# neuronest/custom-alphazero

Measured on AMD Instinct MI355X. Metric: self-play games/s (Connect-4 6x7, 100 sims/move), higher is better.
Workload: dtype fp32-accurate network (fp16 MFMA, two-term split operands, 3 products) / f64 PUCT

## Files before the change

### custom-alphazero_amd/csrc/az_tower16.hip

```cpp
#include <algorithm>
#include <cmath>
#include <cstring>
#include <functional>
#include <type_traits>

#include "az_nn.h"
#include "az_tree.h"
#include "az_kloop_asm.h"
#include "az_chess.h"

namespace az {

typedef _Float16 t_h8 __attribute__((ext_vector_type(8)));
typedef float t_f4 __attribute__((ext_vector_type(4)));

namespace {

constexpr float kRange = 32752.f;
constexpr int kPitch = 544;
constexpr int kZeroRows = 8;
__device__ __forceinline__ bool pix_ok(int yx) { return ((yx >> 8) & 255) != 127; }
__device__ __forceinline__ int pix_row(int yx, int HW, int W) {
  return pix_ok(yx) ? (yx >> 16) * HW + ((yx >> 8) & 255) * W + (yx & 255) : (yx & 7);
}

#ifdef AZ_T16_STAMPS
constexpr int kStampBlocks = 4096, kStamps = 64;
__device__ unsigned long long g_t16_stamps[kStampBlocks][kStamps];
#define T16_STAMP(k)                                                             \
  if (threadIdx.x == 0 && blockIdx.x < kStampBlocks) {                           \
    g_t16_stamps[blockIdx.x][k] = __builtin_amdgcn_s_memtime();                  \
  }
#define T16_RSTAMP(k)                                                            \
  if (threadIdx.x == 0 && blockIdx.x < kStampBlocks) {                           \
    g_t16_stamps[blockIdx.x][k] = __builtin_amdgcn_s_memrealtime();              \
  }
__device__ unsigned long long g_t16_wstamps[kStampBlocks][8][5];
#define T16_WSTAMP(d, k)                                                          \
  if ((d) == 1 && (threadIdx.x & 63) == 0 && blockIdx.x < kStampBlocks) {        \
    g_t16_wstamps[blockIdx.x][threadIdx.x >> 6][k] = __builtin_amdgcn_s_memtime(); \
    if ((k) == 0)                                                                 \
      g_t16_wstamps[blockIdx.x][threadIdx.x >> 6][4] =                            \
          (unsigned)__builtin_amdgcn_s_getreg((31 << 11) | 4);                    \
  }
#define T16_STAMP4(k)                      \
  if (threadIdx.x == 256 && blockIdx.x < kStampBlocks) {                         \
    g_t16_stamps[blockIdx.x][k] = __builtin_amdgcn_s_memtime();                  \
  }
#else
#define T16_STAMP4(k)
#define T16_WSTAMP(d, k)
#define T16_STAMP(k)
#define T16_RSTAMP(k)
#endif

template <typename T>
__device__ __forceinline__ const __attribute__((address_space(1))) T* gbl(const T* p) {
  return (const __attribute__((address_space(1))) T*)p;
}
template <typename T>
__device__ __forceinline__ T gld(const T* p) {
  static_assert(sizeof(T) % 4 == 0, "32-bit words");
  typedef unsigned int V __attribute__((ext_vector_type(sizeof(T) / 4)));
  return __builtin_bit_cast(T, *(const __attribute__((address_space(1))) V*)p);
}


__device__ __forceinline__ void split_u4(const float4 v, uint2& t0, uint2& t1) {
  const float x[4] = {v.x, v.y, v.z, v.w};
  uint32_t p[2], q[2];
#pragma unroll
  for (int i = 0; i < 2; ++i) {
    p[i] = pk_f16(x[2 * i], x[2 * i + 1]);
    const az_h2 h = __builtin_bit_cast(az_h2, p[i]);
    q[i] = pk_f16(x[2 * i] - (float)h[0], x[2 * i + 1] - (float)h[1]);
  }
  t0 = make_uint2(p[0], p[1]);
  t1 = make_uint2(q[0], q[1]);
}
__device__ __forceinline__ void split_u8(const float (&x)[8], uint4& t0, uint4& t1) {
  uint2 a0, a1, b0, b1;
  split_u4(make_float4(x[0], x[1], x[2], x[3]), a0, a1);
  split_u4(make_float4(x[4], x[5], x[6], x[7]), b0, b1);
  t0 = make_uint4(a0.x, a0.y, b0.x, b0.y);
  t1 = make_uint4(a1.x, a1.y, b1.x, b1.y);
}

template <int CTRL>
__device__ __forceinline__ float dpp_f(float v) {
  return __builtin_bit_cast(float, __builtin_amdgcn_update_dpp(0, __builtin_bit_cast(int, v), CTRL, 0xf, 0xf, false));
}
template <typename F>
__device__ __forceinline__ float wreduce(float v, F op) {
  v = op(v, dpp_f<0xB1>(v));
  v = op(v, dpp_f<0x4E>(v));
  v = op(v, dpp_f<0x124>(v));
  v = op(v, dpp_f<0x128>(v));
  const float r0 = __builtin_bit_cast(float, __builtin_amdgcn_readlane(__builtin_bit_cast(int, v), 0));
  const float r1 = __builtin_bit_cast(float, __builtin_amdgcn_readlane(__builtin_bit_cast(int, v), 16));
  const float r2 = __builtin_bit_cast(float, __builtin_amdgcn_readlane(__builtin_bit_cast(int, v), 32));
  const float r3 = __builtin_bit_cast(float, __builtin_amdgcn_readlane(__builtin_bit_cast(int, v), 48));
  return op(op(r0, r1), op(r2, r3));
}
__device__ __forceinline__ float wsum(float v) {
  return wreduce(v, [](float a, float b) { return a + b; });
}
__device__ __forceinline__ float wmax(float v) {
  return wreduce(v, [](float a, float b) { return fmaxf(a, b); });
}

__device__ __forceinline__ int range_exp(float m) {
  int s = 0;
  while (ldexpf(m, -s) > kRange) ++s;
  return s;
}

struct TowerSmem {
  int flag[2];
  int sc[2][kTowerMaxBoards];
  unsigned bmax[kTowerMaxBoards];
};

__device__ __forceinline__ void put4(uint4* act, int r, int cq, const float4 y) {
  uint2 t0, t1;
  split_u4(y, t0, t1);
  char* q = reinterpret_cast<char*>(act) + r * kPitch + cq * 8;
  *reinterpret_cast<uint2*>(q) = t0;
  *reinterpret_cast<uint2*>(q + 256) = t1;
}

__device__ __forceinline__ float max4(const float4 v) { return fmaxf(fmaxf(v.x, v.y), fmaxf(v.z, v.w)); }
__device__ __forceinline__ float4 scale4(const float4 v, float s) {
  return make_float4(v.x * s, v.y * s, v.z * s, v.w * s);
}

template <int MBW>
__device__ __forceinline__ bool store_layer(uint4* act, int HW, int W, const int (&yx_)[MBW], int cq0, const float4 (&y)[2 * MBW],
                                            TowerSmem& sm, int par, int* sc_out, int nbrd,
                                            unsigned long long* err) {
  int row[MBW], brd[MBW];
#pragma unroll
  for (int mb = 0; mb < MBW; ++mb) {
    row[mb] = pix_ok(yx_[mb]) ? pix_row(yx_[mb], HW, W) : -1;
    brd[mb] = yx_[mb] >> 16;
    asm volatile("" : "+v"(row[mb]), "+v"(brd[mb]));
  }
  float vmax = 0.f;
#pragma unroll
  for (int i = 0; i < 2 * MBW; ++i)
    if (row[i / 2] >= 0) {
      vmax = fmaxf(vmax, max4(y[i]));
      put4(act, row[i / 2], cq0 + 4 * (i & 1), y[i]);
    }
  if (!(vmax <= kRange)) sm.flag[par] = 1;
  if (threadIdx.x == 0) sm.flag[par ^ 1] = 0;
  __syncthreads();
  if (!sm.flag[par]) return false;
  if ((int)threadIdx.x < nbrd) sm.bmax[threadIdx.x] = 0u;
  __syncthreads();
#pragma unroll
  for (int i = 0; i < 2 * MBW; ++i)
    if (row[i / 2] >= 0) atomicMax(&sm.bmax[brd[i / 2]], __float_as_uint(max4(y[i])));
  __syncthreads();
#pragma unroll
  for (int i = 0; i < 2 * MBW; ++i) {
    if (row[i / 2] < 0) continue;
    const float m = __uint_as_float(sm.bmax[brd[i / 2]]);
    if (!(m <= 3.0e38f)) continue;
    const int s = range_exp(m);
    if (s) put4(act, row[i / 2], cq0 + 4 * (i & 1), scale4(y[i], ldexpf(1.f, -s)));
  }
  if ((int)threadIdx.x < nbrd) {
    const float m = __uint_as_float(sm.bmax[threadIdx.x]);
    if (!(m <= 3.0e38f)) {
      if (err) atomicOr(err, kErrActRange);
      sc_out[threadIdx.x] = 0;
    } else {
      sc_out[threadIdx.x] = range_exp(m);
    }
  }
  __syncthreads();
  return true;
}

template <int V>
using IC = std::integral_constant<int, V>;

struct NoMid {
  __device__ void operator()() const {}
};
template <int MBW, int R, int C0 = 0, typename Mid = NoMid>
__device__ __forceinline__ void k_loop(const uint4* __restrict__ act, const uint4* __restrict__ wmain,
                                       const uint4* __restrict__ wres, t_f4 (&acc)[MBW][2],
                                       t_f4 (&accr)[MBW][2], const int (&yx_)[MBW], int H, int W,
                                       int zrow, int nq, int lane, int skw, int res_shift = 0,
                                       Mid mid = Mid{}) {
  static_assert(R == 0 || R == 4, "ring slots = k-step mod NB, NB divides 4");
  static_assert(C0 == 0 || (R == 0 && C0 == 2), "skipped chunks: the stem only, an even count");
  constexpr int PF = 1, NB = 2;
  const int gq = lane >> 4;
  int r[MBW], yx[MBW];
#pragma unroll
  for (int mb = 0; mb < MBW; ++mb) {
    yx[mb] = yx_[mb];
    asm volatile("" : "+v"(yx[mb]));
    r[mb] = pix_row(yx[mb], H * W, W);
  }
  uint4 bq[NB][4];
  const auto rs_m = __builtin_amdgcn_make_buffer_rsrc((void*)wmain, (short)0, 0x7fffffff, 0x00020000);
  const auto rs_r = __builtin_amdgcn_make_buffer_rsrc((void*)(R ? wres : wmain), (short)0, 0x7fffffff, 0x00020000);
  const int voff = ((nq * 2) * 2 * 64 + lane) * 16;
  auto load_bk = [&](int s, uint4(&dst)[4]) {
#pragma unroll
    for (int q = 0; q < 4; ++q) {
      const auto v = s < R ? __builtin_amdgcn_raw_buffer_load_b128(rs_r, voff + q * 1024, (36 + s) * 16384, 0)
                           : __builtin_amdgcn_raw_buffer_load_b128(rs_m, voff + q * 1024, (s - R) * 16384, 0);
      dst[q] = __builtin_bit_cast(uint4, v);
    }
  };

  int aaddr[MBW];
  const char* actb = reinterpret_cast<const char*>(act);
  auto set_own = [&](int lo, int hi) {
#pragma unroll
    for (int mb = 0; mb < MBW; ++mb)
      if (mb >= lo && mb < hi) aaddr[mb] = (pix_ok(yx[mb]) ? r[mb] + res_shift : zrow + (r[mb] & 7)) * kPitch + gq * 16;
  };
  auto set_tap = [&](int t, int lo, int hi) {
    const int dy = t / 3 - 1, dx = t - (t / 3) * 3 - 1;
#pragma unroll
    for (int mb = 0; mb < MBW; ++mb) {
      if (mb < lo || mb >= hi) continue;
      const int py = (yx[mb] >> 8) & 255, px = yx[mb] & 255;
      const bool ok = py + dy >= 0 && py + dy < H && px + dx >= 0 && px + dx < W;
      const int sr = r[mb] + dy * W + dx;
      aaddr[mb] = (ok ? sr : zrow + (sr & 7)) * kPitch + gq * 16;
    }
  };
  constexpr int RING = MBW > 4 ? 4 : MBW;
  constexpr bool LAG = RING == MBW && MBW > 1;
  uint4 aq[RING][2];
  auto load_a1 = [&](int chunk, int mb) {
    const char* q = actb + aaddr[mb] + 64 * chunk;
    aq[mb % RING][0] = *reinterpret_cast<const uint4*>(q);
    aq[mb % RING][1] = *reinterpret_cast<const uint4*>(q + 256);
  };
  auto kstep = [&](t_f4(&C)[MBW][2], const uint4(&b)[4], int chunk, int next_chunk, auto skc, auto skn,
                   bool first = false) {
    constexpr int SKC = decltype(skc)::value, SKN = decltype(skn)::value;
    const t_h8 B0[2] = {__builtin_bit_cast(t_h8, b[0]), __builtin_bit_cast(t_h8, b[2])};
    const t_h8 B1[2] = {__builtin_bit_cast(t_h8, b[1]), __builtin_bit_cast(t_h8, b[3])};
#pragma unroll
    for (int mb = 0; mb < MBW; ++mb) {
      const t_h8 a0 = __builtin_bit_cast(t_h8, aq[mb % RING][0]), a1 = __builtin_bit_cast(t_h8, aq[mb % RING][1]);
      if (((SKC >> mb) & 1) == 0) {
#pragma unroll
      for (int nb = 0; nb < 2; ++nb) {
        C[mb][nb] = __builtin_amdgcn_mfma_f32_16x16x32_f16(B0[nb], a1, C[mb][nb], 0, 0, 0);
        C[mb][nb] = __builtin_amdgcn_mfma_f32_16x16x32_f16(B1[nb], a0, C[mb][nb], 0, 0, 0);
        C[mb][nb] = __builtin_amdgcn_mfma_f32_16x16x32_f16(B0[nb], a0, C[mb][nb], 0, 0, 0);
      }
      }
// ... 155 lines not shown
}

#ifdef AZ_KLOOP_CC
#define AZ_KLOOP k_loop
#else
#define AZ_KLOOP k_loop_asm
#endif

template <int NT>
__device__ __forceinline__ void dma_to_lds(uint4* dst, const float* src, int n_u4, int wave, int lane) {
  if (n_u4 <= 0) return;
  const auto rsrc = __builtin_amdgcn_make_buffer_rsrc((void*)src, (short)0, n_u4 * 16, 0x00020000);
  for (int base = wave * 64; base < n_u4; base += NT) {
    const int i = base + lane;
    const unsigned voff = i < n_u4 ? (unsigned)(i * 16) : 0x80000000u;
    __builtin_amdgcn_raw_ptr_buffer_load_lds(rsrc, (__attribute__((address_space(3))) void*)(dst + base), 16,
                                             voff, 0, 0, 0);
  }
}

template <int MBT, int NWM, bool ROWS, bool DB>
__device__ __forceinline__ void tower16_tile(const TowerNet* __restrict__ net, const Board* __restrict__ boards,
                                             const float4* __restrict__ x, const uint4* __restrict__ rows,
                                             int n, int H, int W, int A, int bpw, float* __restrict__ probs,
                                             float* __restrict__ values, float4* __restrict__ feat,
                                             int first_chunk, unsigned long long* __restrict__ err,
                                             TowerLeaves lv) {
  constexpr int MBW = MBT / NWM;
  constexpr int TR = 16 * MBT;
  constexpr int NT = NWM * 256;
  extern __shared__ __attribute__((aligned(16))) uint4 act[];
  const TowerNet& T = *net;
  constexpr bool dbuf = DB;
  uint4* const bufX = act;
  uint4* const bufH = dbuf ? act + (TR + kZeroRows) * (kPitch / 16) : act;
  const int zX = TR, zH = dbuf ? -kZeroRows : TR;
  TowerSmem& sm = *reinterpret_cast<TowerSmem*>(reinterpret_cast<char*>(act) +
                                                ((dbuf ? 2 : 1) * TR + kZeroRows) * kPitch);
  float* blob = reinterpret_cast<float*>(&sm + 1);

  const int HW = H * W;
  const int b0 = blockIdx.x * bpw;
  if (b0 >= n) return;
  const int nbrd = min(bpw, n - b0);
  const int live = nbrd * HW;
  const int tid = threadIdx.x, lane = tid & 63, wave = tid >> 6;
  const int zrow = TR;
  T16_RSTAMP(22);
  T16_STAMP(0);
  const bool alt = 16 * MBT != T.tile_rows && 16 * MBT == T.alt_rows;
  const bool wpd_lds = alt ? T.alt_wpd_lds : T.wpd_lds;
  const bool wv1_lds = alt ? T.alt_wv1_lds : T.wv1_lds;
  const bool wv1_late = alt && wv1_lds;
  dma_to_lds<NT>(reinterpret_cast<uint4*>(blob), T.blob,
                 (wv1_late ? T.off_wv1 : alt ? T.alt_staged_floats : T.staged_floats) / 4, wave, lane);
  for (int i = tid; i < kZeroRows * kPitch / 16; i += NT) act[zrow * kPitch / 16 + i] = make_uint4(0u, 0u, 0u, 0u);
  if (tid < 2) sm.flag[tid] = 0;

  const int mh = wave % NWM, nq = wave / NWM, r16 = lane & 15, gq = lane >> 4;
  const int r0 = mh * MBW * 16 + r16;
  int yx[MBW];
  const bool planned = 16 * MBT == T.tile_rows || alt;
  const bool wv1_xt = T.wv1_xtile && 16 * MBT == T.tile_rows;
  const int* plan = !planned ? nullptr : alt ? T.alt_slot_pix : T.slot_pix;
  T16_STAMP(56);
#pragma unroll
  for (int mb = 0; mb < MBW; ++mb) {
    const int rr = r0 + 16 * mb;
    if (plan) {
      const int v = *gbl(plan + rr);
      yx[mb] = pix_ok(v) && (v >> 16) >= nbrd ? (127 << 8) | (pix_row(v, HW, W) & 7) : v;
    } else {
      const bool valid = rr < live;
      const int b = valid ? rr / HW : 0;
      const int p = rr - b * HW;
      yx[mb] = valid ? (b << 16) | ((p / W) << 8) | (p - (p / W) * W) : (127 << 8) | (rr & 7);
    }
  }
  const int skw = (ROWS && 16 * MBT != 128) ? 0 : !planned ? 0 : alt ? T.alt_skip[mh] : T.skip[mh];
  const int cq0 = 8 * nq + gq;
  t_f4 acc[MBW][2], accr_[MBW][2];
  auto& accr = DB ? acc : accr_;
  float4 yv[2 * MBW];

  if constexpr (ROWS) {
    char* dst = reinterpret_cast<char*>(bufH);
    auto t1_unscale = [](uint32_t w) {
      const az_h2 h = __builtin_bit_cast(az_h2, w);
      return pk_f16((float)h[0] * 0x1p-12f, (float)h[1] * 0x1p-12f);
    };
    if (lv.leaf) {
      const azc::Pos st = azc::start_pos();
      for (int i = tid; i < live * 16; i += NT) {
        const int rr = i >> 4, c4 = 16 + (i & 15), b = rr / HW, pix = rr - b * HW;
        const int s = *gbl(lv.eval_slot + b0 + b);
        const azc::Pos cur = azc::load_pos(static_cast<const az_chess_pos*>(lv.leaf)[s]);
        const bool initial = *gbl(lv.path_len + s) == 0 && *gbl(lv.initial + s) != 0;
        float f[6], v[4];
        azc::state_feats(cur, f);
        azc::full_state4(st, cur, initial, f, pix, 4 * c4, v);
        uint2 t0, t1;
        split16x4(make_float4(v[0], v[1], v[2], v[3]), t0, t1);
        char* q = dst + rr * kPitch;
        *reinterpret_cast<uint2*>(q + 8 * c4) = t0;
        *reinterpret_cast<uint2*>(q + 256 + 8 * c4) = make_uint2(t1_unscale(t1.x), t1_unscale(t1.y));
      }
    } else {
      const uint4* src = rows + (size_t)b0 * HW * 32;
#pragma unroll 4
      for (int i = tid; i < live * 32; i += NT) {
        uint4 v = gld(src + i);
        if ((i & 31) >= 16) v = make_uint4(t1_unscale(v.x), t1_unscale(v.y), t1_unscale(v.z), t1_unscale(v.w));
        *reinterpret_cast<uint4*>(dst + (i >> 5) * kPitch + (i & 31) * 16) = v;
      }
    }
#pragma unroll
    for (int mb = 0; mb < MBW; ++mb)
#pragma unroll
      for (int nb = 0; nb < 2; ++nb) acc[mb][nb] = t_f4{0.f, 0.f, 0.f, 0.f};
    __builtin_amdgcn_s_waitcnt(0);
    __syncthreads();
    if (first_chunk == 2) AZ_KLOOP<MBW, 0, 2>(bufH, T.stem_k, nullptr, acc, acc, yx, H, W, zH, nq, lane, skw);
    else AZ_KLOOP<MBW, 0, 0>(bufH, T.stem_k, nullptr, acc, acc, yx, H, W, zH, nq, lane, skw);
    if (!dbuf) __syncthreads();
  } else {
  {
    const uint4* ws = T.stem16 + (size_t)(nq * 2) * 2 * 64 + lane;
    uint4 bs2[2][4];
#pragma unroll
    for (int ks = 0; ks < 2; ++ks)
#pragma unroll
      for (int q = 0; q < 4; ++q) bs2[ks][q] = gld(ws + (size_t)ks * 1024 + q * 64);
#pragma unroll
    for (int mb = 0; mb < MBW; ++mb)
#pragma unroll
      for (int nb = 0; nb < 2; ++nb) acc[mb][nb] = t_f4{0.f, 0.f, 0.f, 0.f};
    constexpr int SG = MBW <= 4 ? MBW : MBW % 4 == 0 ? 4 : MBW % 3 == 0 ? 3 : 1;
    static_assert(MBW % SG == 0, "stem groups");
#pragma unroll
    for (int g0 = 0; g0 < MBW; g0 += SG) {
      Board bd[SG];
      if (boards) {
#pragma unroll
        for (int i = 0; i < SG; ++i) bd[i] = gld(boards + b0 + (yx[g0 + i] >> 16));
      }
#pragma unroll
      for (int ks = 0; ks < 2; ++ks) {
        const uint4(&bs)[4] = bs2[ks];
        const t_h8 B0[2] = {__builtin_bit_cast(t_h8, bs[0]), __builtin_bit_cast(t_h8, bs[2])};
        const t_h8 B1[2] = {__builtin_bit_cast(t_h8, bs[1]), __builtin_bit_cast(t_h8, bs[3])};
#pragma unroll
        for (int i = 0; i < SG; ++i) {
          const int mb = g0 + i;
          float v[8];
#pragma unroll
          for (int h = 0; h < 2; ++h) {
            const int t = 8 * ks + 2 * gq + h;
            const int dy = t / 3 - 1, dx = t - (t / 3) * 3 - 1;
            const int py = (yx[mb] >> 8) & 255, px = yx[mb] & 255;
            const bool ok = t < 9 && py + dy >= 0 && py + dy < H && px + dx >= 0 && px + dx < W;
            float4 pl = make_float4(0.f, 0.f, 0.f, 0.f);
            if (ok) {
              const int q = (py + dy) * W + px + dx;
              if (boards) {
                const uint64_t ow = q < 64 ? bd[i].own[0] : bd[i].own[1],
                               op = q < 64 ? bd[i].opp[0] : bd[i].opp[1];
                const bool o = (ow >> (q & 63)) & 1ull, e = (op >> (q & 63)) & 1ull;
                pl = make_float4(o || e ? 0.f : 1.f, o ? 1.f : 0.f, e ? 1.f : 0.f, 1.f);
              } else {
                pl = gld(x + (size_t)(b0 + (yx[mb] >> 16)) * HW + q);
              }
            }
            v[4 * h + 0] = pl.x;
            v[4 * h + 1] = pl.y;
            v[4 * h + 2] = pl.z;
            v[4 * h + 3] = pl.w;
          }
          uint4 a0, a1;
          split_u8(v, a0, a1);
#pragma unroll
          for (int nb = 0; nb < 2; ++nb) {
            acc[mb][nb] = __builtin_amdgcn_mfma_f32_16x16x32_f16(B0[nb], __builtin_bit_cast(t_h8, a1), acc[mb][nb], 0, 0, 0);
            acc[mb][nb] = __builtin_amdgcn_mfma_f32_16x16x32_f16(B1[nb], __builtin_bit_cast(t_h8, a0), acc[mb][nb], 0, 0, 0);
            acc[mb][nb] = __builtin_amdgcn_mfma_f32_16x16x32_f16(B0[nb], __builtin_bit_cast(t_h8, a0), acc[mb][nb], 0, 0, 0);
          }
        }
      }
    }
  }
  T16_STAMP(57);
  __builtin_amdgcn_s_waitcnt(0);
  T16_STAMP(58);
  __syncthreads();
  }
  T16_STAMP(1);
  {
    const float osc = ROWS ? T.stem_ks : T.stem_s;
    const float* bb = blob + T.off_stemb;
#pragma unroll
    for (int nb = 0; nb < 2; ++nb) {
      const float4 bc = *reinterpret_cast<const float4*>(bb + 32 * nq + 16 * nb + 4 * gq);
#pragma unroll
      for (int mb = 0; mb < MBW; ++mb) {
        const t_f4 a = acc[mb][nb];
        yv[mb * 2 + nb] = make_float4(fmaxf(fmaf(a[0], osc, bc.x), 0.f), fmaxf(fmaf(a[1], osc, bc.y), 0.f),
                                      fmaxf(fmaf(a[2], osc, bc.z), 0.f), fmaxf(fmaf(a[3], osc, bc.w), 0.f));
      }
    }
  }
  int par = 0;
  bool anyX = store_layer<MBW>(bufX, HW, W, yx, cq0, yv, sm, par, sm.sc[0], nbrd, err);
  bool anyH = false;
  float* red = nullptr;
  const int J = T.hidden;
  par ^= 1;
  T16_STAMP(21);

  const int depth = T.depth;
  for (int d = 0; d < depth; ++d) {
#pragma unroll
    for (int mb = 0; mb < MBW; ++mb)
#pragma unroll
      for (int nb = 0; nb < 2; ++nb) {
        acc[mb][nb] = t_f4{0.f, 0.f, 0.f, 0.f};
        accr_[mb][nb] = t_f4{0.f, 0.f, 0.f, 0.f};
      }
    T16_WSTAMP(d, 0);
    if constexpr (DB) AZ_KLOOP<MBW, 0, 0>(bufX, T.k1[d], nullptr, acc, acc, yx, H, W, zX, nq, lane, skw);
    else AZ_KLOOP<MBW, 4, 0>(bufX, T.k1[d], T.k2[d], acc, accr_, yx, H, W, zX, nq, lane, skw);
    T16_WSTAMP(d, 1);
    if (d < 4) T16_STAMP(2 + 4 * d);
    if (d < 4) T16_STAMP4(24 + 4 * d);
    if (!dbuf) __syncthreads();
    if (d < 4) T16_STAMP(40 + d);
    {
      const float osc = T.s1[d];
      const float* bb = blob + T.off_b1 + d * 128;
#pragma unroll
      for (int nb = 0; nb < 2; ++nb) {
        const float4 bc = *reinterpret_cast<const float4*>(bb + 32 * nq + 16 * nb + 4 * gq);
#pragma unroll
        for (int mb = 0; mb < MBW; ++mb) {
          const float o = anyX ? ldexpf(osc, sm.sc[0][yx[mb] >> 16]) : osc;
          const t_f4 a = acc[mb][nb];
          yv[mb * 2 + nb] = make_float4(fmaxf(fmaf(a[0], o, bc.x), 0.f), fmaxf(fmaf(a[1], o, bc.y), 0.f),
                                        fmaxf(fmaf(a[2], o, bc.z), 0.f), fmaxf(fmaf(a[3], o, bc.w), 0.f));
        }
      }
    }
    anyH = store_layer<MBW>(bufH, HW, W, yx, cq0, yv, sm, par, sm.sc[1], nbrd, err);
    par ^= 1;
    if (d < 4) T16_STAMP(3 + 4 * d);
    auto rescale = [&]() {
      if (anyX || anyH) {
#pragma unroll
        for (int mb = 0; mb < MBW; ++mb) {
          const int e = (anyX ? sm.sc[0][yx[mb] >> 16] : 0) - (anyH ? sm.sc[1][yx[mb] >> 16] : 0);
          if (e) {
            const float f = ldexpf(1.f, e);
#pragma unroll
            for (int nb = 0; nb < 2; ++nb) accr[mb][nb] *= f;
          }
        }
      }
    };
    T16_WSTAMP(d, 2);
    if constexpr (DB) {
      const bool wv1x = (wv1_xt || wv1_late) && d + 1 == depth;
      auto mid = [&]() {
        rescale();
        __syncthreads();
        if (wv1x)
          dma_to_lds<NT>(reinterpret_cast<uint4*>(wv1_xt ? reinterpret_cast<float*>(bufX) + TR * 48 : blob + T.off_wv1),
                         T.blob + T.off_wv1, (HW * J + 3) / 4, wave, lane);
      };
#pragma unroll
      for (int mb = 0; mb < MBW; ++mb)
#pragma unroll
        for (int nb = 0; nb < 2; ++nb) acc[mb][nb] = t_f4{0.f, 0.f, 0.f, 0.f};
      AZ_KLOOP<MBW, 4, 0>(bufH, T.k2[d], T.k2[d], acc, acc, yx, H, W, zH, nq, lane, skw, -(TR + kZeroRows),
                            mid);
    } else {
      rescale();
      AZ_KLOOP<MBW, 0, 0>(bufH, T.k2[d], nullptr, accr, accr, yx, H, W, zH, nq, lane, skw);
    }
    T16_WSTAMP(d, 3);
    if (d < 4) T16_STAMP(4 + 4 * d);
    if (d < 4) T16_STAMP4(26 + 4 * d);
    const float osc = T.s2[d];
    const float* bb = blob + T.off_b2 + d * 128;
    if (d + 1 < depth) {
      if (!dbuf) __syncthreads();
#pragma unroll
      for (int nb = 0; nb < 2; ++nb) {
        const float4 bc = *reinterpret_cast<const float4*>(bb + 32 * nq + 16 * nb + 4 * gq);
#pragma unroll
        for (int mb = 0; mb < MBW; ++mb) {
          const float o = anyH ? ldexpf(osc, sm.sc[1][yx[mb] >> 16]) : osc;
          const t_f4 a = accr[mb][nb];
          yv[mb * 2 + nb] = make_float4(fmaxf(fmaf(a[0], o, bc.x), 0.f), fmaxf(fmaf(a[1], o, bc.y), 0.f),
                                        fmaxf(fmaf(a[2], o, bc.z), 0.f), fmaxf(fmaf(a[3], o, bc.w), 0.f));
        }
      }
      anyX = store_layer<MBW>(bufX, HW, W, yx, cq0, yv, sm, par, sm.sc[0], nbrd, err);
      par ^= 1;
      if (d < 4) T16_STAMP(5 + 4 * d);
      continue;
    }
    if (dbuf) {
      red = reinterpret_cast<float*>(bufX);
    } else {
      __syncthreads();
      red = reinterpret_cast<float*>(act);
    }
    const float* wpc = blob + T.off_wpc;
    const float* wvc = blob + T.off_wvc;
    int hr[MBW], hyx[MBW], hb[MBW];
#pragma unroll
    for (int mb = 0; mb < MBW; ++mb) {
      hr[mb] = pix_row(yx[mb], HW, W);
      hyx[mb] = yx[mb];
      hb[mb] = yx[mb] >> 16;
      asm volatile("" : "+v"(hr[mb]), "+v"(hyx[mb]), "+v"(hb[mb]));
    }
    int hq = 32 * nq + 4 * gq;
    asm volatile("" : "+v"(hq));
    T16_STAMP4(48);
    float bcv[2][4], wp[2][4][2], wv[2][4];
#pragma unroll
    for (int nb = 0; nb < 2; ++nb) {
      const int c0 = hq + 16 * nb;
      const float4 bc = *reinterpret_cast<const float4*>(bb + c0);
      const float4 p01 = *reinterpret_cast<const float4*>(wpc + 2 * c0);
      const float4 p23 = *reinterpret_cast<const float4*>(wpc + 2 * c0 + 4);
      const float4 vv = *reinterpret_cast<const float4*>(wvc + c0);
      const float bq[4] = {bc.x, bc.y, bc.z, bc.w}, pq[8] = {p01.x, p01.y, p01.z, p01.w, p23.x, p23.y, p23.z, p23.w},
                  vq[4] = {vv.x, vv.y, vv.z, vv.w};
#pragma unroll
      for (int v = 0; v < 4; ++v) {
        bcv[nb][v] = bq[v];
        wp[nb][v][0] = pq[2 * v];
        wp[nb][v][1] = pq[2 * v + 1];
        wv[nb][v] = vq[v];
      }
    }
#pragma unroll
    for (int mb = 0; mb < MBW; ++mb) {
      T16_STAMP4(49 + mb);
      const float o = anyH ? ldexpf(osc, sm.sc[1][hb[mb]]) : osc;
      float a0 = 0.f, a1 = 0.f, a2 = 0.f;
#pragma unroll
      for (int nb = 0; nb < 2; ++nb) {
#pragma unroll
        for (int v = 0; v < 4; ++v) {
          const float yy = fmaxf(fmaf(accr[mb][nb][v], o, bcv[nb][v]), 0.f);
          a0 = fmaf(yy, wp[nb][v][0], a0);
          a1 = fmaf(yy, wp[nb][v][1], a1);
          a2 = fmaf(yy, wv[nb][v], a2);
        }
      }
      if (pix_ok(hyx[mb])) {
        float* q = red + (hr[mb] * 16 + nq * 4 + gq) * 3;
        q[0] = a0;
        q[1] = a1;
        q[2] = a2;
      }
    }
  }
  T16_STAMP4(54);
  T16_STAMP(42);
  T16_STAMP4(43);
  if (wv1_xt || wv1_late) __builtin_amdgcn_s_waitcnt(0);
  __syncthreads();
  T16_STAMP(18);
  if constexpr (ROWS) {
    const float* hbias = blob + T.off_hb;
    const float bpc0 = hbias[0], bpc1 = hbias[1], bvc0 = hbias[2];
    for (int rr = tid; rr < live; rr += NT) {
      const float* q = red + rr * 48;
      float t[3] = {0.f, 0.f, 0.f};
#pragma unroll
      for (int j = 0; j < 16; ++j)
#pragma unroll
        for (int k = 0; k < 3; ++k) t[k] += q[3 * j + k];
      feat[(size_t)b0 * HW + rr] =
          make_float4(fmaxf(t[0] + bpc0, 0.f), fmaxf(t[1] + bpc1, 0.f), fmaxf(t[2] + bvc0, 0.f), 0.f);
    }
    return;
  }

  const int P = NT / J;
  float* pf = dbuf ? reinterpret_cast<float*>(bufH) : red + TR * 48;
  float* vf = pf + ((bpw * 2 * HW + 3) & ~3);
  float* lg = vf + kTowerMaxBoards * HW;
  float* pp = lg + bpw * A;
  float* vp = pp + NT;
  float* hv = vp + bpw * P * J;
  {
    const float* hbias = blob + T.off_hb;
    const float bpc0 = hbias[0], bpc1 = hbias[1], bvc0 = hbias[2];
    for (int i = tid; i < 3 * live; i += NT) {
      const int rr = i / 3, k = i - 3 * rr;
      const float* q = red + rr * 48 + k;
      float t = 0.f;
#pragma unroll
      for (int j = 0; j < 16; ++j) t += q[3 * j];
      const int b = rr / HW, p = rr - b * HW;
      if (k < 2) pf[b * 2 * HW + 2 * p + k] = fmaxf(t + (k ? bpc1 : bpc0), 0.f);
      else vf[p * kTowerMaxBoards + b] = fmaxf(t + bvc0, 0.f);
    }
  }
  __syncthreads();
  T16_STAMP(44);
  {
    const int K = 2 * HW, O = nbrd * A, OP = NT / 16;
    const float* bpd = blob + T.off_bpd;
    const float* bv1 = blob + T.off_bv1;
    const float* wv2 = blob + T.off_wv2;
    auto policy_part = [&](int base, auto wpd) {
      const int o = base + tid / 16, pi = tid & 15;
      float sacc = 0.f;
      if (o < O) {
        const int b = o / A, a = o - b * A;
        const float* pb = pf + b * K;
        for (int k0 = pi; k0 < K; k0 += 64) {
          float xv[4], wv[4];
#pragma unroll
          for (int u = 0; u < 4; ++u) {
            const int k = k0 + 16 * u;
            xv[u] = k < K ? pb[k] : 0.f;
            wv[u] = k < K ? wpd[k * A + a] : 0.f;
          }
#pragma unroll
          for (int u = 0; u < 4; ++u) sacc = fmaf(xv[u], wv[u], sacc);
        }
      }
      pp[tid] = sacc;
    };
    auto value_part_n = [&](auto wv1, auto nbv) {
      constexpr int NBV = decltype(nbv)::value;
      const int j = tid % J, q = tid / J;
      if (q >= P) return;
      float sv[NBV];
#pragma unroll
      for (int b = 0; b < NBV; ++b) sv[b] = 0.f;
      for (int p0 = q; p0 < HW; p0 += 4 * P) {
        float w[4], v[4][NBV];
#pragma unroll
        for (int u = 0; u < 4; ++u) {
          const int p = p0 + u * P;
          const int pc = p < HW ? p : 0;
          w[u] = p < HW ? wv1[pc * J + j] : 0.f;
#pragma unroll
          for (int h = 0; h < NBV / 4; ++h) {
            const float4 f = *reinterpret_cast<const float4*>(vf + pc * kTowerMaxBoards + 4 * h);
            v[u][4 * h] = f.x, v[u][4 * h + 1] = f.y, v[u][4 * h + 2] = f.z, v[u][4 * h + 3] = f.w;
          }
        }
#pragma unroll
        for (int u = 0; u < 4; ++u)
#pragma unroll
          for (int b = 0; b < NBV; ++b) sv[b] = fmaf(v[u][b], w[u], sv[b]);
      }
#pragma unroll
      for (int b = 0; b < NBV; ++b)
        if (b < nbrd) vp[(b * P + q) * J + j] = sv[b];
    };
    auto value_part = [&](auto wv1) {
      if (nbrd <= 4) value_part_n(wv1, IC<4>{});
      else value_part_n(wv1, IC<kTowerMaxBoards>{});
    };
    for (int base = 0;; base += OP) {
      if (wpd_lds) policy_part(base, blob + T.off_wpd);
      else policy_part(base, gbl(T.blob + T.off_wpd));
      if (base == 0) {
        if (wv1_lds) value_part(blob + T.off_wv1);
        else if (wv1_xt) value_part(reinterpret_cast<const float*>(bufX) + TR * 48);
        else value_part(gbl(T.blob + T.off_wv1));
      }
      if (base == 0) T16_STAMP(45);
      __syncthreads();
      if (base == 0) T16_STAMP(46);
      if (tid < OP && base + tid < O) {
        const int o = base + tid, a = o % A;
        float t = 0.f;
#pragma unroll
        for (int j = 0; j < 16; ++j) t += pp[tid * 16 + j];
        lg[o] = t + bpd[a];
      }
      if (base == 0) {
        for (int i = tid; i < nbrd * J; i += NT) {
          const int b = i / J, j = i - b * J;
          float t = 0.f;
          for (int q = 0; q < P; ++q) t += vp[(b * P + q) * J + j];
          hv[i] = fmaxf(t + bv1[j], 0.f) * wv2[j];
        }
      }
      if (base == 0) T16_STAMP(47);
      __syncthreads();
      if (base + OP >= O) break;
    }
  }
  const float bv2 = blob[T.off_hb + 3];
  for (int b = wave; b < nbrd; b += NT / 64) {
    float m = -INFINITY;
    for (int a = lane; a < A; a += 64) m = fmaxf(m, lg[b * A + a]);
    m = wmax(m);
    float z = 0.f;
    for (int a = lane; a < A; a += 64) z += expf(lg[b * A + a] - m);
    z = wsum(z);
    for (int a = lane; a < A; a += 64) probs[(size_t)(b0 + b) * A + a] = expf(lg[b * A + a] - m) / z;
    float v = 0.f;
    for (int j = lane; j < J; j += 64) v += hv[b * J + j];
    v = wsum(v);
    if (lane == 0) values[b0 + b] = tanhf(v + bv2);
  }
  T16_STAMP(19);
  T16_RSTAMP(23);
}

template <int MBT, int NWM, bool ROWS, bool DB>
__global__ __launch_bounds__(NWM * 256, NWM) void tower16_kernel(const TowerNet* __restrict__ net,
                                                               const Board* __restrict__ boards,
                                                               const float4* __restrict__ x,
                                                               const uint4* __restrict__ rows,
                                                               const int* __restrict__ count, int n_static,
                                                               int H, int W, int A, int bpw,
                                                               float* __restrict__ probs,
                                                               float* __restrict__ values,
                                                               float4* __restrict__ feat, int first_chunk,
                                                               unsigned long long* __restrict__ err,
                                                               TowerLeaves lv) {
  tower16_tile<MBT, NWM, ROWS, DB>(net, boards, x, rows, count ? *count : n_static, H, W, A, bpw, probs, values,
                                   feat, first_chunk, err, lv);
}

template <int MBT, int MBT2, bool DB>
__global__ __launch_bounds__(512, 2) void tower16_dual_kernel(const TowerNet* __restrict__ net,
                                                              const Board* __restrict__ boards,
                                                              const float4* __restrict__ x,
                                                              const int* __restrict__ count, int n_static,
                                                              int H, int W, int A, int bpw, int bpw2,
                                                              float* __restrict__ probs, float* __restrict__ values,
                                                              unsigned long long* __restrict__ err) {
  const int n = count ? *count : n_static;
  if (n <= net->alt_max_boards)
    tower16_tile<MBT2, 2, false, DB>(net, boards, x, nullptr, n, H, W, A, bpw2, probs, values, nullptr, 0, err, {});
  else
    tower16_tile<MBT, 2, false, DB>(net, boards, x, nullptr, n, H, W, A, bpw, probs, values, nullptr, 0, err, {});
}

}

#ifdef AZ_T16_STAMPS
}
extern "C" int az_t16_stamps(unsigned long long* out) {
  return hipMemcpyFromSymbol(out, HIP_SYMBOL(az::g_t16_stamps), sizeof(az::g_t16_stamps)) == hipSuccess ? 0 : -1;
}
extern "C" int az_t16_wstamps(unsigned long long* out) {
  return hipMemcpyFromSymbol(out, HIP_SYMBOL(az::g_t16_wstamps), sizeof(az::g_t16_wstamps)) == hipSuccess ? 0 : -1;
}
namespace az {
#endif

int tower16_tile_rows(int HW) {
  if (HW > 128) return 0;
  if (HW > 64 && HW <= 96) return 192;
  const int b128 = std::min(128 / HW, kTowerMaxBoards), b96 = std::min(96 / HW, kTowerMaxBoards);
  if (b96 >= 1 && b96 * HW * 128 >= b128 * HW * 96) return 96;
  return 128;
}

int tower16_boards_per_tile(int HW, int tr) { return tr ? std::min(tr / HW, kTowerMaxBoards) : 0; }

size_t tower16_lds_bytes(int HW, int tr, int staged_floats, bool dbuf) {
  (void)HW;
  return (size_t)((dbuf ? 2 : 1) * tr + kZeroRows) * kPitch + sizeof(TowerSmem) + (size_t)staged_floats * sizeof(float);
}

bool tower16_heads_fit(int HW, int tr, int A, int hidden, bool dbuf) {
  const int bpw = tower16_boards_per_tile(HW, tr), nt = 512;
  if (!tr || hidden < 1 || hidden > 256) return false;
  const int p = nt / hidden;
  const size_t need = (size_t)bpw * 2 * HW + 3 + (size_t)kTowerMaxBoards * HW + (size_t)bpw * A + nt +
                      (size_t)bpw * p * hidden + (size_t)bpw * hidden;
  const size_t have = (size_t)tr * (kPitch / 4) - (dbuf ? 0 : (size_t)tr * 48);
  return need <= have;
}

bool tower16_wv1_xtile_fits(int HW, int tr, int hidden) {
  return tr && (HW * hidden) % 4 == 0 && (size_t)tr * 48 * 4 + (size_t)HW * hidden * 4 <= (size_t)tr * kPitch;
}

namespace {
struct PlanBorder {
  int cls, blk;
};

bool slot_plan_try(int H, int W, int tr, const std::vector<PlanBorder>& borders, std::vector<int>& slot_pix,
                   int skip[2]) {
  const int HW = H * W, nb = tower16_boards_per_tile(HW, tr), nblk = tr / 16, half = nblk / 2;
  auto cls = [&](int y, int x, int c) {
    return c == 0 ? y == 0 : c == 1 ? x == 0 : c == 2 ? y == H - 1 : x == W - 1;
  };
  const int nbor = (int)borders.size();
  std::vector<int> interior;
  for (int k = 0; k < nblk; ++k) {
    bool b = false;
    for (const PlanBorder& e : borders) b = b || e.blk == k;
    if (!b) interior.push_back(k);
  }
  const int nint = (int)interior.size();
  const int S1[8] = {0, 1, 2, 3, 12, 13, 14, 15}, S2[8] = {4, 5, 6, 7, 8, 9, 10, 11};
  const int kEmpty = 127 << 8;
  std::vector<int> slot(tr, -1);
  auto word = [&](int n) { return ((n / HW) << 16) | (((n % HW) / W) << 8) | (n % W); };
  std::vector<int> overflow;
  for (int r = 0; r < 8; ++r) {
    std::vector<int> P;
    for (int n = r; n < nb * HW; n += 8) P.push_back(n);
    const int ns = 2 * nbor;
    std::vector<int> owner(ns, -1);
    std::function<bool(int, std::vector<char>&)> aug = [&](int pi, std::vector<char>& seen) {
      const int n = P[pi], y = (n % HW) / W, x = n % W;
      for (int sl = 0; sl < ns; ++sl) {
        if (seen[sl] || !cls(y, x, borders[sl / 2].cls)) continue;
        seen[sl] = 1;
        if (owner[sl] < 0 || aug(owner[sl], seen)) {
          owner[sl] = pi;
          return true;
        }
      }
      return false;
    };
    for (int pi = 0; pi < (int)P.size(); ++pi) {
      std::vector<char> seen(ns, 0);
      aug(pi, seen);
    }
    std::vector<char> used(P.size(), 0);
    for (int sl = 0; sl < ns; ++sl) {
      const int at = borders[sl / 2].blk * 16 + ((sl & 1) ? S2[r] : S1[r]);
      if (owner[sl] >= 0) {
        slot[at] = word(P[owner[sl]]);
        used[owner[sl]] = 1;
      } else {
        slot[at] = kEmpty | r;
      }
    }
    int k = 0;
    for (int pi = 0; pi < (int)P.size(); ++pi) {
      if (used[pi]) continue;
      if (k < 2 * nint) {
        slot[interior[k / 2] * 16 + ((k & 1) ? S2[r] : S1[r])] = word(P[pi]);
        ++k;
      } else {
        overflow.push_back(P[pi]);
      }
    }
    for (; k < 2 * nint; ++k) slot[interior[k / 2] * 16 + ((k & 1) ? S2[r] : S1[r])] = -2 - r;
  }
  for (int n : overflow) {
    bool placed = false;
    for (int j = 0; j < tr && !placed; ++j)
      if (slot[j] <= -2) {
        slot[j] = word(n);
        placed = true;
      }
    if (!placed) return false;
// ... 214 lines not shown
```

### profiles/tower_stamps.py

```python
import ctypes
import os
import sys

import numpy as np

REPO = os.path.dirname(os.path.dirname(os.path.abspath(__file__)))
sys.path.insert(0, os.path.join(REPO, "custom-alphazero_amd"))
sys.path.insert(0, os.path.join(REPO, "oracle"))
import oracle
from custom_alphazero import engine as az
from custom_alphazero.model.weights import init_weights, weight_spec


def main():
    nb = int(sys.argv[1]) if len(sys.argv) > 1 else 673
    rng = np.random.RandomState(5)
    w = init_weights(weight_spec(6, 7, 7, depth=4), seed=0, randomize_bn=True)
    eng = az.Engine(6, 7, 4, True, 25, slots=max(nb, 2048), evaluator=az.EVAL_NETWORK, depth=4)
    eng.set_weights(w.items())
    xx = oracle.full_state(rng.randint(-1, 2, (nb, 6, 7)).astype(np.int8))
    for _ in range(30):
        eng.forward(xx)
    buf = np.zeros((4096, 64), np.uint64)
    lib = az.load_library()
    lib.az_t16_stamps.argtypes = [ctypes.c_void_p]
    assert lib.az_t16_stamps(buf.ctypes.data) == 0
    nwg = (nb + 2) // 3
    s = buf[:nwg].astype(np.int64)
    rel = s - s[:, 0:1]
    clk = (s[:, 19] - s[:, 0]) / np.maximum((s[:, 23] - s[:, 22]) / 100.0, 1)
    order = [(0, "start"), (1, "stem mfma"), (21, "stem store")]
    for d in range(4):
        for k, p in enumerate(("c1loop", "c1epi", "c2loop", "c2epi")):
            if not (d == 3 and p == "c2epi"):
                order.append((2 + 4 * d + k, f"b{d}.{p}"))
    order += [(18, "heads1x1"), (19, "end")]
    med = np.median(rel, axis=0)
    prev = 0
    print(f"B={nb} wgs={nwg} clock {np.median(clk):.0f} MHz; total {med[19]:.0f} cycles")
    for i, n in order:
        print(f"  {n:10s} {med[i]:9.0f}  (+{med[i] - prev:7.0f})")
        prev = med[i]
    print(f"  stem: before plan {med[56]:.0f}, MFMAs issued {med[57]:.0f}, DMA landed {med[58]:.0f}, barrier {med[1]:.0f}")
    print("  wave4 1x1: " + " ".join(f"{med[k]:.0f}" for k in range(48, 56)))
    print(f"  heads: pf/vf {med[44]:.0f}, policy {med[45]:.0f}, value {med[46]:.0f}, barrier {med[47]:.0f}, "
          f"end {med[19]:.0f}; last conv2 wave0 {med[16]:.0f} wave4 {med[38]:.0f}; 1x1 done wave0 {med[42]:.0f} "
          f"wave4 {med[43]:.0f}")
    for d in range(4):
        print(f"  b{d}: wave4 c1loop end {med[24 + 4 * d]:.0f} (wave0 {med[2 + 4 * d]:.0f}), after barrier "
              f"{med[40 + d]:.0f}, c1epi end {med[3 + 4 * d]:.0f}; wave4 c2loop end {med[26 + 4 * d]:.0f} "
              f"(wave0 {med[4 + 4 * d]:.0f})")
    if hasattr(lib, "az_t16_wstamps"):
        ws = np.zeros((4096, 8, 5), np.uint64)
        lib.az_t16_wstamps.argtypes = [ctypes.c_void_p]
        assert lib.az_t16_wstamps(ws.ctypes.data) == 0
        ws = ws[:nwg].astype(np.int64)
        t0 = ws[:, :, 0].min(axis=1, keepdims=True)
        simd = (ws[:, :, 4] >> 4) & 3
        print("  block 1 per wave (median over workgroups, cycles from the first wave's conv1 start):")
        for w in range(8):
            c1s, c1e, c2s, c2e = (np.median(ws[:, w, k] - t0[:, 0]) for k in range(4))
            sid = np.bincount(simd[:, w], minlength=4).argmax()
            print(f"    wave {w} simd {sid}: conv1 {c1s:7.0f}..{c1e:7.0f} ({c1e - c1s:6.0f})  "
                  f"conv2 {c2s:7.0f}..{c2e:7.0f} ({c2e - c2s:6.0f})")


if __name__ == "__main__":
    main()
```

Baseline: 11400.

## Streamline stem board planes and fuse head reductions into single pass

The board-input stem now builds fp16 one-hot planes directly as bit patterns with a zero low-order split, instead of going through a float split. It also skips the empty tap slot. In the heads, integer divisions become reciprocal-multiply divisions, and the policy weight loads are issued before the value dense computation so their latency is hidden. When all outputs fit in one pass, a barrier and the separate logits/hidden round trip through LDS are removed, and softmax and value sums run per wave straight from partials. The added code paths raise complexity, and the float-reciprocal division could be inexact for larger operands.

```diff
diff --git a/custom-alphazero_amd/csrc/az_tower16.hip b/custom-alphazero_amd/csrc/az_tower16.hip
--- a/custom-alphazero_amd/csrc/az_tower16.hip
+++ b/custom-alphazero_amd/csrc/az_tower16.hip
@@ -108,6 +108,8 @@
 __device__ __forceinline__ float wmax(float v) {
   return wreduce(v, [](float a, float b) { return fmaxf(a, b); });
 }
+
+__device__ __forceinline__ int div_small(int n, float rd) { return (int)(((float)n + 0.5f) * rd); }
 
 __device__ __forceinline__ int range_exp(float m) {
   int s = 0;
@@ -569,32 +571,43 @@
 #pragma unroll
         for (int i = 0; i < SG; ++i) {
           const int mb = g0 + i;
-          float v[8];
-#pragma unroll
-          for (int h = 0; h < 2; ++h) {
-            const int t = 8 * ks + 2 * gq + h;
-            const int dy = t / 3 - 1, dx = t - (t / 3) * 3 - 1;
-            const int py = (yx[mb] >> 8) & 255, px = yx[mb] & 255;
-            const bool ok = t < 9 && py + dy >= 0 && py + dy < H && px + dx >= 0 && px + dx < W;
-            float4 pl = make_float4(0.f, 0.f, 0.f, 0.f);
-            if (ok) {
-              const int q = (py + dy) * W + px + dx;
-              if (boards) {
-                const uint64_t ow = q < 64 ? bd[i].own[0] : bd[i].own[1],
-                               op = q < 64 ? bd[i].opp[0] : bd[i].opp[1];
-                const bool o = (ow >> (q & 63)) & 1ull, e = (op >> (q & 63)) & 1ull;
-                pl = make_float4(o || e ? 0.f : 1.f, o ? 1.f : 0.f, e ? 1.f : 0.f, 1.f);
-              } else {
-                pl = gld(x + (size_t)(b0 + (yx[mb] >> 16)) * HW + q);
+          const int py = (yx[mb] >> 8) & 255, px = yx[mb] & 255;
+          uint4 a0, a1;
+          if (boards) {
+            uint32_t wd[2][2];
+#pragma unroll
+            for (int h = 0; h < 2; ++h) {
+              wd[h][0] = wd[h][1] = 0u;
+              if (ks == 1 && h == 1) continue;
+              const int t = 8 * ks + 2 * gq + h;
+              const int dy = t / 3 - 1, dx = t - (t / 3) * 3 - 1;
+              const int qy = py + dy, qx = px + dx, q = qy * W + qx;
+              const bool ok = t < 9 && (unsigned)qy < (unsigned)H && (unsigned)qx < (unsigned)W;
+              const uint64_t ow = q < 64 ? bd[i].own[0] : bd[i].own[1], op = q < 64 ? bd[i].opp[0] : bd[i].opp[1];
+              const uint32_t o = (uint32_t)(ow >> (q & 63)) & 1u, e = (uint32_t)(op >> (q & 63)) & 1u;
+              if (ok) {
+                wd[h][0] = ((o | e) ? 0u : 0x3c00u) | (o ? 0x3c000000u : 0u);
+                wd[h][1] = (e ? 0x3c00u : 0u) | 0x3c000000u;
               }
             }
-            v[4 * h + 0] = pl.x;
-            v[4 * h + 1] = pl.y;
-            v[4 * h + 2] = pl.z;
-            v[4 * h + 3] = pl.w;
+            a0 = make_uint4(wd[0][0], wd[0][1], wd[1][0], wd[1][1]);
+            a1 = make_uint4(0u, 0u, 0u, 0u);
+          } else {
+            float v[8];
+#pragma unroll
+            for (int h = 0; h < 2; ++h) {
+              const int t = 8 * ks + 2 * gq + h;
+              const int dy = t / 3 - 1, dx = t - (t / 3) * 3 - 1;
+              const bool ok = t < 9 && py + dy >= 0 && py + dy < H && px + dx >= 0 && px + dx < W;
+              float4 pl = make_float4(0.f, 0.f, 0.f, 0.f);
+              if (ok) pl = gld(x + (size_t)(b0 + (yx[mb] >> 16)) * HW + (py + dy) * W + px + dx);
+              v[4 * h + 0] = pl.x;
+              v[4 * h + 1] = pl.y;
+              v[4 * h + 2] = pl.z;
+              v[4 * h + 3] = pl.w;
+            }
+            split_u8(v, a0, a1);
           }
-          uint4 a0, a1;
-          split_u8(v, a0, a1);
 #pragma unroll
           for (int nb = 0; nb < 2; ++nb) {
             acc[mb][nb] = __builtin_amdgcn_mfma_f32_16x16x32_f16(B0[nb], __builtin_bit_cast(t_h8, a1), acc[mb][nb], 0, 0, 0);
@@ -634,6 +647,8 @@
   T16_STAMP(21);
 
   const int depth = T.depth;
+  const int off_b2 = T.off_b2, off_wpc = T.off_wpc, off_wvc = T.off_wvc, off_hb = T.off_hb, off_bpd = T.off_bpd,
+            off_bv1 = T.off_bv1, off_wv2 = T.off_wv2, off_wpd = T.off_wpd, off_wv1 = T.off_wv1;
   for (int d = 0; d < depth; ++d) {
 #pragma unroll
     for (int mb = 0; mb < MBW; ++mb)
@@ -681,6 +696,7 @@
         }
       }
     };
+    const float osc = T.s2[d];
     T16_WSTAMP(d, 2);
     if constexpr (DB) {
       const bool wv1x = (wv1_xt || wv1_late) && d + 1 == depth;
@@ -688,8 +704,8 @@
         rescale();
         __syncthreads();
         if (wv1x)
-          dma_to_lds<NT>(reinterpret_cast<uint4*>(wv1_xt ? reinterpret_cast<float*>(bufX) + TR * 48 : blob + T.off_wv1),
-                         T.blob + T.off_wv1, (HW * J + 3) / 4, wave, lane);
+          dma_to_lds<NT>(reinterpret_cast<uint4*>(wv1_xt ? reinterpret_cast<float*>(bufX) + TR * 48 : blob + off_wv1),
+                         T.blob + off_wv1, (HW * J + 3) / 4, wave, lane);
       };
 #pragma unroll
       for (int mb = 0; mb < MBW; ++mb)
@@ -704,8 +720,7 @@
     T16_WSTAMP(d, 3);
     if (d < 4) T16_STAMP(4 + 4 * d);
     if (d < 4) T16_STAMP4(26 + 4 * d);
-    const float osc = T.s2[d];
-    const float* bb = blob + T.off_b2 + d * 128;
+    const float* bb = blob + off_b2 + d * 128;
     if (d + 1 < depth) {
       if (!dbuf) __syncthreads();
 #pragma unroll
@@ -730,8 +745,8 @@
       __syncthreads();
       red = reinterpret_cast<float*>(act);
     }
-    const float* wpc = blob + T.off_wpc;
-    const float* wvc = blob + T.off_wvc;
+    const float* wpc = blob + off_wpc;
+    const float* wvc = blob + off_wvc;
     int hr[MBW], hyx[MBW], hb[MBW];
 #pragma unroll
     for (int mb = 0; mb < MBW; ++mb) {
@@ -791,7 +806,7 @@
   __syncthreads();
   T16_STAMP(18);
   if constexpr (ROWS) {
-    const float* hbias = blob + T.off_hb;
+    const float* hbias = blob + off_hb;
     const float bpc0 = hbias[0], bpc1 = hbias[1], bvc0 = hbias[2];
     for (int rr = tid; rr < live; rr += NT) {
       const float* q = red + rr * 48;
@@ -806,7 +821,9 @@
     return;
   }
 
-  const int P = NT / J;
+  const float rHW = __builtin_amdgcn_rcpf((float)HW), rA = __builtin_amdgcn_rcpf((float)A),
+              rJ = __builtin_amdgcn_rcpf((float)J);
+  const int P = div_small(NT, rJ);
   float* pf = dbuf ? reinterpret_cast<float*>(bufH) : red + TR * 48;
   float* vf = pf + ((bpw * 2 * HW + 3) & ~3);
   float* lg = vf + kTowerMaxBoards * HW;
@@ -814,7 +831,7 @@
   float* vp = pp + NT;
   float* hv = vp + bpw * P * J;
   {
-    const float* hbias = blob + T.off_hb;
+    const float* hbias = blob + off_hb;
     const float bpc0 = hbias[0], bpc1 = hbias[1], bvc0 = hbias[2];
     for (int i = tid; i < 3 * live; i += NT) {
       const int rr = i / 3, k = i - 3 * rr;
@@ -822,46 +839,56 @@
       float t = 0.f;
 #pragma unroll
       for (int j = 0; j < 16; ++j) t += q[3 * j];
-      const int b = rr / HW, p = rr - b * HW;
+      const int b = div_small(rr, rHW), p = rr - b * HW;
       if (k < 2) pf[b * 2 * HW + 2 * p + k] = fmaxf(t + (k ? bpc1 : bpc0), 0.f);
       else vf[p * kTowerMaxBoards + b] = fmaxf(t + bvc0, 0.f);
     }
   }
   __syncthreads();
   T16_STAMP(44);
+  const int K = 2 * HW, O = nbrd * A, OP = NT / 16;
+  const float* bpd = blob + off_bpd;
+  const float* bv1 = blob + off_bv1;
+  const float* wv2 = blob + off_wv2;
+  const float bv2 = blob[off_hb + 3];
   {
-    const int K = 2 * HW, O = nbrd * A, OP = NT / 16;
-    const float* bpd = blob + T.off_bpd;
-    const float* bv1 = blob + T.off_bv1;
-    const float* wv2 = blob + T.off_wv2;
-    auto policy_part = [&](int base, auto wpd) {
-      const int o = base + tid / 16, pi = tid & 15;
-      float sacc = 0.f;
-      if (o < O) {
-        const int b = o / A, a = o - b * A;
-        const float* pb = pf + b * K;
-        for (int k0 = pi; k0 < K; k0 += 64) {
-          float xv[4], wv[4];
-#pragma unroll
-          for (int u = 0; u < 4; ++u) {
-            const int k = k0 + 16 * u;
-            xv[u] = k < K ? pb[k] : 0.f;
-            wv[u] = k < K ? wpd[k * A + a] : 0.f;
-          }
-#pragma unroll
-          for (int u = 0; u < 4; ++u) sacc = fmaf(xv[u], wv[u], sacc);
-        }
-      }
-      pp[tid] = sacc;
-    };
+    const int pl = tid >> 4, pi = tid & 15;
+    const int vq = div_small(tid, rJ), vj = tid - vq * J;
     auto value_part_n = [&](auto wv1, auto nbv) {
       constexpr int NBV = decltype(nbv)::value;
-      const int j = tid % J, q = tid / J;
+      const int j = vj, q = vq;
       if (q >= P) return;
       float sv[NBV];
 #pragma unroll
       for (int b = 0; b < NBV; ++b) sv[b] = 0.f;
-      for (int p0 = q; p0 < HW; p0 += 4 * P) {
+      const int PJ = P * J;
+      int p0 = q;
+      auto whole = [&](auto nu) {
+        constexpr int NU = decltype(nu)::value;
+        float w[NU], v[NU][NBV];
+        const int iw = p0 * J + j;
+        const float* pv = vf + p0 * kTowerMaxBoards;
+#pragma unroll
+        for (int u = 0; u < NU; ++u) {
+          w[u] = wv1[iw + u * PJ];
+#pragma unroll
+          for (int h = 0; h < NBV / 4; ++h) {
+            const float4 f = *reinterpret_cast<const float4*>(pv + u * P * kTowerMaxBoards + 4 * h);
+            v[u][4 * h] = f.x, v[u][4 * h + 1] = f.y, v[u][4 * h + 2] = f.z, v[u][4 * h + 3] = f.w;
+          }
+        }
+#pragma unroll
+        for (int u = 0; u < NU; ++u)
+#pragma unroll
+          for (int b = 0; b < NBV; ++b) sv[b] = fmaf(v[u][b], w[u], sv[b]);
+      };
+      if constexpr (NBV == 4) {
+#pragma unroll 1
+        for (; p0 + 7 * P < HW; p0 += 8 * P) whole(IC<8>{});
+      }
+#pragma unroll 1
+      for (; p0 + 3 * P < HW; p0 += 4 * P) whole(IC<4>{});
+      if (p0 < HW) {
         float w[4], v[4][NBV];
 #pragma unroll
         for (int u = 0; u < 4; ++u) {
@@ -883,23 +910,72 @@
       for (int b = 0; b < NBV; ++b)
         if (b < nbrd) vp[(b * P + q) * J + j] = sv[b];
     };
-    auto value_part = [&](auto wv1) {
-      if (nbrd <= 4) value_part_n(wv1, IC<4>{});
-      else value_part_n(wv1, IC<kTowerMaxBoards>{});
+    auto value_part = [&]() {
+      auto by_boards = [&](auto wv1) {
+        if (nbrd <= 4) value_part_n(wv1, IC<4>{});
+        else value_part_n(wv1, IC<kTowerMaxBoards>{});
+      };
+      if (wv1_lds || wv1_xt) by_boards(wv1_lds ? blob + off_wv1 : reinterpret_cast<const float*>(bufX) + TR * 48);
+      else by_boards(gbl(T.blob + off_wv1));
     };
+    auto policy_part = [&](int base) {
+      const int o = base + pl;
+      const bool on = o < O;
+      const int b = div_small(on ? o : 0, rA), a = (on ? o : 0) - b * A;
+      const float* pb = pf + b * K;
+      const bool slice = K <= 128;
+      float sacc = 0.f, xv[8], wv[8];
+      auto reads = [&](auto wpd) {
+#pragma unroll
+        for (int u = 0; u < 8; ++u) {
+          const int k = pi + 16 * u;
+          const bool in = on && k < K;
+          xv[u] = in ? pb[k] : 0.f;
+          wv[u] = in ? wpd[k * A + a] : 0.f;
+        }
+      };
+      auto batches = [&](auto wpd) {
+        for (int k0 = pi; k0 < K; k0 += 64) {
+          float x4[4], w4[4];
+#pragma unroll
+          for (int u = 0; u < 4; ++u) {
+            const int k = k0 + 16 * u;
+            x4[u] = k < K ? pb[k] : 0.f;
+            w4[u] = k < K ? wpd[k * A + a] : 0.f;
+          }
+#pragma unroll
+          for (int u = 0; u < 4; ++u) sacc = fmaf(x4[u], w4[u], sacc);
+        }
+      };
+      if (slice) {
+        if (wpd_lds) reads(blob + off_wpd);
+        else reads(gbl(T.blob + off_wpd));
+      }
+      if (base == 0) value_part();
+      if (slice) {
+        if (on) {
+#pragma unroll
+          for (int u = 0; u < 4; ++u) sacc = fmaf(xv[u], wv[u], sacc);
+          if (pi + 64 < K) {
+#pragma unroll
+            for (int u = 4; u < 8; ++u) sacc = fmaf(xv[u], wv[u], sacc);
+          }
+        }
+      } else if (on) {
+        if (wpd_lds) batches(blob + off_wpd);
+        else batches(gbl(T.blob + off_wpd));
+      }
+      pp[tid] = sacc;
+    };
+    const bool one_pass = O <= OP && nbrd <= NT / 128;
     for (int base = 0;; base += OP) {
-      if (wpd_lds) policy_part(base, blob + T.off_wpd);
-      else policy_part(base, gbl(T.blob + T.off_wpd));
-      if (base == 0) {
-        if (wv1_lds) value_part(blob + T.off_wv1);
-        else if (wv1_xt) value_part(reinterpret_cast<const float*>(bufX) + TR * 48);
-        else value_part(gbl(T.blob + T.off_wv1));
-      }
+      policy_part(base);
       if (base == 0) T16_STAMP(45);
       __syncthreads();
       if (base == 0) T16_STAMP(46);
+      if (one_pass) break;
       if (tid < OP && base + tid < O) {
-        const int o = base + tid, a = o % A;
+        const int o = base + tid, a = o - div_small(o, rA) * A;
         float t = 0.f;
 #pragma unroll
         for (int j = 0; j < 16; ++j) t += pp[tid * 16 + j];
@@ -907,7 +983,7 @@
       }
       if (base == 0) {
         for (int i = tid; i < nbrd * J; i += NT) {
-          const int b = i / J, j = i - b * J;
+          const int b = div_small(i, rJ), j = i - b * J;
           float t = 0.f;
           for (int q = 0; q < P; ++q) t += vp[(b * P + q) * J + j];
           hv[i] = fmaxf(t + bv1[j], 0.f) * wv2[j];
@@ -917,20 +993,58 @@
       __syncthreads();
       if (base + OP >= O) break;
     }
-  }
-  const float bv2 = blob[T.off_hb + 3];
-  for (int b = wave; b < nbrd; b += NT / 64) {
-    float m = -INFINITY;
-    for (int a = lane; a < A; a += 64) m = fmaxf(m, lg[b * A + a]);
-    m = wmax(m);
-    float z = 0.f;
-    for (int a = lane; a < A; a += 64) z += expf(lg[b * A + a] - m);
-    z = wsum(z);
-    for (int a = lane; a < A; a += 64) probs[(size_t)(b0 + b) * A + a] = expf(lg[b * A + a] - m) / z;
-    float v = 0.f;
-    for (int j = lane; j < J; j += 64) v += hv[b * J + j];
-    v = wsum(v);
-    if (lane == 0) values[b0 + b] = tanhf(v + bv2);
+    if (one_pass) {
+      T16_STAMP(47);
+      if (wave < nbrd) {
+        const bool on = lane < A;
+        float l = -INFINITY;
+        if (on) {
+          const float* q = pp + (wave * A + lane) * 16;
+          float t = 0.f;
+#pragma unroll
+          for (int j = 0; j < 16; ++j) t += q[j];
+          l = t + bpd[lane];
+        }
+        const float m = wmax(fmaxf(-INFINITY, l));
+        const float e = on ? expf(l - m) : 0.f;
+        const float z = wsum(0.f + e);
+        if (on) probs[(size_t)(b0 + wave) * A + lane] = e / z;
+      } else if (wave >= NT / 128 && wave - NT / 128 < nbrd) {
+#pragma clang fp contract(off)
+        const int b = wave - NT / 128;
+        float t[4] = {0.f, 0.f, 0.f, 0.f};
+#pragma unroll 1
+        for (int q = 0; q < P; ++q) {
+          const float* pq = vp + (b * P + q) * J + lane;
+#pragma unroll
+          for (int i = 0; i < 4; ++i)
+            if (lane + 64 * i < J) t[i] += pq[64 * i];
+        }
+        float v = 0.f;
+#pragma unroll
+        for (int i = 0; i < 4; ++i)
+          if (lane + 64 * i < J) {
+            const float h = fmaxf(t[i] + bv1[lane + 64 * i], 0.f) * wv2[lane + 64 * i];
+            v += h;
+          }
+        v = wsum(v);
+        if (lane == 0) values[b0 + b] = tanhf(v + bv2);
+      }
+    } else {
+      for (int b = wave; b < nbrd; b += NT / 64) {
+        float m = -INFINITY;
+        for (int a = lane; a < A; a += 64) m = fmaxf(m, lg[b * A + a]);
+        m = wmax(m);
+        float z = 0.f;
+        for (int a = lane; a < A; a += 64) z += expf(lg[b * A + a] - m);
+        z = wsum(z);
+        for (int a = lane; a < A; a += 64) probs[(size_t)(b0 + b) * A + a] = expf(lg[b * A + a] - m) / z;
+        float v = 0.f;
+        for (int j = lane; j < J; j += 64) v += hv[b * J + j];
+        v = wsum(v);
+        if (lane == 0) values[b0 + b] = tanhf(v + bv2);
+      }
+    }
   }
   T16_STAMP(19);
   T16_RSTAMP(23);
diff --git a/profiles/tower_stamps.py b/profiles/tower_stamps.py
--- a/profiles/tower_stamps.py
+++ b/profiles/tower_stamps.py
@@ -43,7 +43,7 @@
         prev = med[i]
     print(f"  stem: before plan {med[56]:.0f}, MFMAs issued {med[57]:.0f}, DMA landed {med[58]:.0f}, barrier {med[1]:.0f}")
     print("  wave4 1x1: " + " ".join(f"{med[k]:.0f}" for k in range(48, 56)))
-    print(f"  heads: pf/vf {med[44]:.0f}, policy {med[45]:.0f}, value {med[46]:.0f}, barrier {med[47]:.0f}, "
+    print(f"  heads: pf/vf {med[44]:.0f}, dense {med[45]:.0f}, dense barrier {med[46]:.0f}, sums {med[47]:.0f}, "
           f"end {med[19]:.0f}; last conv2 wave0 {med[16]:.0f} wave4 {med[38]:.0f}; 1x1 done wave0 {med[42]:.0f} "
           f"wave4 {med[43]:.0f}")
     for d in range(4):
```

Result: faster. 11550 (median of 6 runs) (+1.4%).
